# ml-jku/LaM-SLidE

Hardware: AMD Instinct MI355X
Metric: sampled trajectories/sec (50-step ODE) + decoded-coord L2 vs ref, MD17 (higher is better)
Workload: dtype bf16; 1 GPU; md17_bench; tail=False, ln_fuse=True, T=30, L=256, C=32, D=512, H=16, depth=4, sampler=ODE, state_updates=50, batch_per_gpu=32, global_batch=32, parallelism=batch-shard x1, 1 gather to rank 0 per step, noise_elem_stride_per_rank=7864320, kernels=general, trajectories_per_pass=32

## Files before the change

### lam_slide_amd/csrc/k_lin1.hip.h

```cpp
#pragma once
#include <type_traits>

#include "common.hip.h"

struct Lin1Args {
    const u16 *W;
    const u16 *X;
    const float *bias;
    const float4 *rope_q, *rope_k;
    u16 *qkv;
    u16 *z;
    int F, N, HHD, M;
    int pos_div, pos_mod;
    unsigned div_magic, mod_magic;
    float inv_hd, q_premul;
    int nt;
    int wpt;
    int planes;
    int npad;
    const float2 *ln_stat;
    const float *ln_shift, *ln_scale;
    int ln_mod_stride, ln_tpt;
    unsigned ln_tpt_magic;
};

#ifndef LIN1_B2
#define LIN1_B2 1
#endif
#ifndef LIN1_B2_KMAX
#define LIN1_B2_KMAX 256
#endif

template <int HDP, int K, int NW = 8>
struct Lin1Cfg {
    static_assert(K % 128 == 0 && K <= 512, "hidden sizes 128 / 256 / 384 / 512");
    static constexpr int KS = K / 16;
    static constexpr int ROWB = 2 * K;
    static constexpr int PITCH = ROWB + 16;
    static constexpr int BLK = 32 * PITCH;
    static constexpr int NS = (LIN1_B2 && K <= LIN1_B2_KMAX) ? 4 : 3;
    static constexpr int RING = NS * BLK;
    static_assert(NW == 8 || NW == 4, "two waves per SIMD (256-token tiles) or one (128-token tiles)");
    static constexpr int TT = 32 * NW;
    static constexpr int STAGE = NW * 4096;
    static constexpr int LPR = ROWB / 16;
    static constexpr int PPW = 32 / NW;
    static constexpr size_t lds_bytes(int F) { return (size_t)RING + STAGE + (size_t)F * 4; }
    static constexpr int LN_SLOTS = K <= 256 ? 3 : 2;
    static constexpr size_t lds_bytes_lnf(int F) { return lds_bytes(F) + (size_t)LN_SLOTS * 2 * K * 4; }
};

enum { LIN1_QK = 0, LIN1_V = 1, LIN1_MLP = 2 };

#ifndef LIN1_XLOAD
#define LIN1_XLOAD 1
#endif
#ifndef LIN1_PD
#define LIN1_PD 3
#endif

__device__ __forceinline__ float lin1_gelu(float x) {
    const float ax = fabsf(x);
    const float h = __builtin_amdgcn_exp2f(LSL_GELU_Q(ax));
    float relu;
    asm("v_max_f32 %0, 0, %1" : "=v"(relu) : "v"(x));
    return fmaf(-ax, h, relu);
}

template <int HDP, int K, int NW = 8, bool LNF = false>
__global__ void __launch_bounds__(NW * 64, NW / 4) k_linear1_ts(Lin1Args g) {
    using C = Lin1Cfg<HDP, K, NW>;
    constexpr int KS = C::KS, BLK = C::BLK, PPW = C::PPW, ROWB = C::ROWB;
    constexpr int NCO = HDP == 32 ? 8 : 4;
    extern __shared__ __attribute__((aligned(16))) char smem[];

    const int tid = threadIdx.x, lane = tid & 63;
    const int wave = __builtin_amdgcn_readfirstlane(tid >> 6);
    const int r = lane & 31, hf = lane >> 5;
    char *const stage = smem + C::RING + wave * 4096;
    float *const bias_lds = reinterpret_cast<float *>(smem + C::RING + C::STAGE);

    const int NB = g.F >> 5;
    const int ntile = (g.N + C::TT - 1) / C::TT;
    const long U = (long)ntile * NB;
    long i0, i1;
    if (g.wpt > 0) {
        const int tile = blockIdx.x / g.wpt, part = blockIdx.x - tile * g.wpt;
        i0 = (long)tile * NB + ((NB * part / g.wpt) & ~1);
        i1 = (long)tile * NB + (part + 1 == g.wpt ? NB : ((NB * (part + 1) / g.wpt) & ~1));
    } else {
        i0 = (U * blockIdx.x / gridDim.x) & ~1L;
        i1 = blockIdx.x + 1 == gridDim.x ? U : ((U * (blockIdx.x + 1) / gridDim.x) & ~1L);
    }
    if (i0 >= i1) return;

    for (int i = tid * 4; i < g.F; i += NW * 64 * 4) *reinterpret_cast<float4 *>(bias_lds + i) = *reinterpret_cast<const float4 *>(g.bias + i);

    const unsigned lds0 = (unsigned)(size_t)(LDS_PTR(char))(smem);
    const unsigned lane_src = lane * 16;
    const char *const w_rows = reinterpret_cast<const char *>(g.W) + (size_t)(PPW * wave) * ROWB;
    auto issue_piece = [&](const char *src, unsigned dst, auto ic) __attribute__((always_inline)) {
        constexpr int I = decltype(ic)::value & 3;
        if (decltype(ic)::value >= 4) {
            src += 4 * ROWB;
            dst += 4 * C::PITCH;
        }
        const unsigned ls = lane_src;
        if (C::LPR == 64 || lane < C::LPR) {
            if (I == 0 || decltype(ic)::value >= 4)
                asm volatile("s_add_u32 m0, %2, %3\n\ts_nop 4\n\tglobal_load_lds_dwordx4 %0, %1 offset:%4" ::"v"(ls), "s"(src), "s"(dst), "n"(16 * I), "n"(ROWB * I) : "memory", "scc");
            else
                asm volatile("s_add_u32 m0, %2, %3\n\ts_nop 0\n\tglobal_load_lds_dwordx4 %0, %1 offset:%4" ::"v"(ls), "s"(src), "s"(dst), "n"(16 * I), "n"(ROWB * I) : "memory", "scc");
        }
    };
    auto req_src = [&](int blk) __attribute__((always_inline)) { return w_rows + (size_t)blk * (32 * ROWB); };
    auto req_dst = [&](int slot) __attribute__((always_inline)) { return lds0 + slot * BLK + PPW * wave * C::PITCH; };
    auto issue = [&](int blk, int slot) __attribute__((always_inline)) {
        const char *src = req_src(blk);
        const unsigned dst = req_dst(slot);
        issue_piece(src, dst, std::integral_constant<int, 0>());
        issue_piece(src, dst, std::integral_constant<int, 1>());
        issue_piece(src, dst, std::integral_constant<int, 2>());
        issue_piece(src, dst, std::integral_constant<int, 3>());
        if (PPW == 8) {
            issue_piece(src, dst, std::integral_constant<int, 4>());
            issue_piece(src, dst, std::integral_constant<int, 5>());
            issue_piece(src, dst, std::integral_constant<int, 6>());
            issue_piece(src, dst, std::integral_constant<int, 7>());
        }
    };
    const int aoff = r * C::PITCH + 16 * hf;

    bf16x8 xreg[KS];
    float4 co[NCO];
    f32x16 acc0, acc1;
    int slot_c = 0;
    int dma_blk, dma_slot;
    int n_wave = 0;
    float post = 1.0f;

    auto advance = [&](int &b) __attribute__((always_inline)) { b = b + 1 == NB ? 0 : b + 1; };
    auto next_slot = [&](int s) __attribute__((always_inline)) { return s == C::NS - 1 ? 0 : s + 1; };

    {
        int b = (int)(i0 - (i0 / NB) * NB);
        issue(b, 0);
        advance(b);
        issue(b, 1);
        advance(b);
        dma_blk = b;
        dma_slot = 2;
    }

    auto init_acc = [&](f32x16 &a, int blk) __attribute__((always_inline)) {
#pragma unroll
        for (int q4 = 0; q4 < 4; ++q4) {
            const float4 b = *reinterpret_cast<const float4 *>(bias_lds + blk * 32 + 8 * q4 + 4 * hf);
            a[4 * q4] = b.x; a[4 * q4 + 1] = b.y; a[4 * q4 + 2] = b.z; a[4 * q4 + 3] = b.w;
        }
    };
    constexpr bool B2 = LIN1_B2 != 0 && K <= LIN1_B2_KMAX;
    auto step_head = [&](auto flushed_c) __attribute__((always_inline)) {
        if (B2) {
            if (decltype(flushed_c)::value) wait_vmcnt<PPW>();
            else wait_vmcnt<0>();
        } else {
            if (decltype(flushed_c)::value) wait_vmcnt<PPW + 4>();
            else wait_vmcnt<PPW>();
        }
        __builtin_amdgcn_s_barrier();
        asm volatile("" ::: "memory");
    };
    const unsigned wr0 = (unsigned)(size_t)(LDS_PTR(char))(stage) + r * 128 + 8 * hf + ((r & 7) << 4);
    const unsigned rd0 = (unsigned)(size_t)(LDS_PTR(char))(stage) + (lane >> 3) * 128 + (((lane & 7) ^ ((lane >> 3) & 7)) << 4);
    const char *row_q = nullptr, *row_z = nullptr;
    const bool planes = g.planes != 0;
    constexpr unsigned PROW = 2u * HDP, CPH = HDP / 8;
    const unsigned plane_bytes = PROW * (unsigned)g.npad;
    const unsigned stride_q = planes ? PROW : 2u * 3 * g.HHD, stride_z = 2u * (g.HHD + g.M);
    const unsigned blk_q = planes ? (32 / HDP) * plane_bytes : 64u;
    const unsigned voff_q = planes ? ((lane & 7) / CPH) * plane_bytes + (lane >> 3) * PROW + 16 * ((lane & 7) % CPH) : (lane >> 3) * stride_q + 16 * (lane & 7);
    const unsigned voff_z = (lane >> 3) * stride_z + 16 * (lane & 7);
    const int slab_z = 3 * (g.HHD >> 5);
    const char *fl_base = nullptr;
    unsigned fl_stride8 = 0, fl_voff = 0;
    auto flush_setup = [&](int b_even) __attribute__((always_inline)) {
        const bool to_qkv = b_even < slab_z;
        fl_base = to_qkv ? row_q : row_z;
        fl_stride8 = 8 * (to_qkv ? stride_q : stride_z);
        fl_voff = to_qkv ? voff_q + blk_q * (unsigned)b_even : voff_z + 64u * (unsigned)b_even;
    };
    auto flush_read = [&](int half, u32x4 (&pk)[2]) __attribute__((always_inline)) {
#pragma unroll
        for (int i = 0; i < 2; ++i) pk[i] = *reinterpret_cast<const LDS_PTR(u32x4)>(rd0 + 1024 * (2 * half + i));
    };
    auto flush_store = [&](int half, const u32x4 (&pk)[2]) __attribute__((always_inline)) {
        asm volatile("s_nop 4\n\tglobal_store_dwordx4 %0, %1, %2 nt\n\ts_nop 1" ::"v"(fl_voff + (2 * half) * fl_stride8), "v"(pk[0]), "s"(fl_base) : "memory");
        asm volatile("global_store_dwordx4 %0, %1, %2 nt\n\ts_nop 1" ::"v"(fl_voff + (2 * half + 1) * fl_stride8), "v"(pk[1]), "s"(fl_base) : "memory");
    };
    auto flush_store_visible = [&](int half, const u32x4 (&pk)[2]) __attribute__((always_inline)) {
#pragma unroll
        for (int i = 0; i < 2; ++i)
            __builtin_nontemporal_store(pk[i], reinterpret_cast<u32x4 *>(const_cast<char *>(fl_base) + (size_t)(fl_voff + (2 * half + i) * fl_stride8)));
    };
    auto put_group = [&](int ii, int q, float v0, float v1, float v2, float v3) __attribute__((always_inline)) {
        const u32x2 pk = {pack2(v0, v1), pack2(v2, v3)};
        *reinterpret_cast<LDS_PTR(u32x2)>(wr0 ^ (unsigned)(64 * ii + 16 * q)) = pk;
    };
    auto epi_slice = [&](auto sec_c, int s, const f32x16 &a, int ii, float &c0, float &c1) __attribute__((always_inline)) {
        constexpr int SEC = decltype(sec_c)::value;
        if constexpr (SEC == LIN1_QK && HDP == 32) {
            if (s == 0) c0 = 0.0f;
            if (s < 2) {
#pragma unroll
                for (int e = 0; e < 8; ++e) c0 = fmaf(a[8 * s + e], a[8 * s + e], c0);
            }
            if (s == 1) c0 = rsqrtf(fmaf(half_pair_sum(c0), g.inv_hd, 1e-6f)) * post;
            if (s >= 2 && s < 6) {
                const int q = s - 2;
                float o[4];
#pragma unroll
                for (int kk = 0; kk < 2; ++kk) {
                    const int k = 2 * q + kk;
                    const float x0 = a[2 * k], x1 = a[2 * k + 1];
                    o[2 * kk] = c0 * fmaf(co[k].x, x0, -co[k].y * x1);
                    o[2 * kk + 1] = c0 * fmaf(co[k].z, x0, co[k].w * x1);
                }
                put_group(ii, q, o[0], o[1], o[2], o[3]);
            }
        } else if constexpr (SEC == LIN1_QK) {
            if (s == 0) {
                c0 = 0.0f;
#pragma unroll
                for (int e = 0; e < 8; ++e) c0 = fmaf(a[e], a[e], c0);
            }
            if (s == 1) {
                c1 = 0.0f;
#pragma unroll
                for (int e = 0; e < 8; ++e) c1 = fmaf(a[8 + e], a[8 + e], c1);
                c0 = rsqrtf(fmaf(half_pair_sum(c0), g.inv_hd, 1e-6f)) * post;
                c1 = rsqrtf(fmaf(half_pair_sum(c1), g.inv_hd, 1e-6f)) * post;
            }
            if (s >= 2 && s < 6) {
                const int q = s - 2;
                const float rr = q < 2 ? c0 : c1;
                float o[4];
#pragma unroll
                for (int kk = 0; kk < 2; ++kk) {
                    const int k = 2 * q + kk;
                    const float x0 = a[2 * k], x1 = a[2 * k + 1];
                    const float4 cf = co[k & (NCO - 1)];
                    o[2 * kk] = rr * fmaf(cf.x, x0, -cf.y * x1);
                    o[2 * kk + 1] = rr * fmaf(cf.z, x0, cf.w * x1);
                }
                put_group(ii, q, o[0], o[1], o[2], o[3]);
            }
        } else if constexpr (SEC == LIN1_MLP) {
            const float g0 = lin1_gelu(a[2 * s]), g1 = lin1_gelu(a[2 * s + 1]);
            if (s & 1) put_group(ii, s >> 1, c0, c1, g0, g1);
            else { c0 = g0; c1 = g1; }
        } else {
            if (s < 4) put_group(ii, s, a[4 * s], a[4 * s + 1], a[4 * s + 2], a[4 * s + 3]);
        }
    };
    auto step = [&](auto sec_c, auto par_c, auto mfma_c, auto epi_c, auto side) __attribute__((always_inline)) {
        constexpr int PAR = decltype(par_c)::value;
        constexpr bool DO_MFMA = decltype(mfma_c)::value != 0, DO_EPI = decltype(epi_c)::value != 0;
        constexpr int MPS = KS / 8, PD = LIN1_PD, MH = (MPS + 1) / 2;
        f32x16 &ac = PAR ? acc0 : acc1;
        const f32x16 &ae = PAR ? acc1 : acc0;
        const char *sb = smem + slot_c * BLK + aoff;
        bf16x8 fr[PD];
        float c0 = 0.0f, c1 = 0.0f;
        if (DO_MFMA) {
#pragma unroll
            for (int ks = 0; ks < PD; ++ks) fr[ks] = as_bf16x8(*reinterpret_cast<const u32x4 *>(sb + 32 * ks));
        }
        side(std::integral_constant<int, -1>());
#define LIN1_SIDE(S) if (s == S) side(std::integral_constant<int, S>());
#pragma unroll
        for (int s = 0; s < 8; ++s) {
#pragma unroll
            for (int m = 0; m < MPS; ++m) {
                if (m == MH) { LIN1_SIDE(0) LIN1_SIDE(1) LIN1_SIDE(2) LIN1_SIDE(3) LIN1_SIDE(4) LIN1_SIDE(5) LIN1_SIDE(6) LIN1_SIDE(7) }
                if (DO_MFMA) {
                    const int ks = s * MPS + m;
                    ac = mfma32(fr[ks % PD], xreg[ks], ac);
                    if (ks + PD < KS) fr[ks % PD] = as_bf16x8(*reinterpret_cast<const u32x4 *>(sb + 32 * (ks + PD)));
                }
            }
            if (MH == MPS) { LIN1_SIDE(0) LIN1_SIDE(1) LIN1_SIDE(2) LIN1_SIDE(3) LIN1_SIDE(4) LIN1_SIDE(5) LIN1_SIDE(6) LIN1_SIDE(7) }
            if (DO_EPI) epi_slice(sec_c, s, ae, PAR, c0, c1);
            __builtin_amdgcn_sched_barrier(0);
        }
#undef LIN1_SIDE
        if (decltype(mfma_c)::value != 0) slot_c = next_slot(slot_c);
    };
    std::integral_constant<int, 0> I0;
    std::integral_constant<int, 1> I1;
    auto no_side = [](auto) __attribute__((always_inline)) {};
    auto fused = [&](auto sec_c, auto par_c, auto flush_c, auto prev_c, int e) __attribute__((always_inline)) {
        constexpr int PAR = decltype(par_c)::value;
        constexpr bool FLUSH = decltype(flush_c)::value != 0;
        if (!B2 || PAR == 1) step_head(prev_c);
        u32x4 pk[2];
        if (FLUSH) flush_setup(e - 2);
        const char *src = req_src(dma_blk);
        const unsigned dst = req_dst(dma_slot);
        int blk2 = dma_blk;
        advance(blk2);
        const char *src2 = req_src(blk2);
        const unsigned dst2 = req_dst(next_slot(dma_slot));
        init_acc(PAR ? acc0 : acc1, e + 1);
        step(sec_c, par_c, I1, I1, [&](auto sl) __attribute__((always_inline)) {
            constexpr int SL = decltype(sl)::value;
            if (FLUSH) {
                if (SL == -1) flush_read(0, pk);
                if (SL == 0) {
                    flush_store(0, pk);
                    flush_read(1, pk);
                }
                if (SL == 1) flush_store(1, pk);
            }
            constexpr int PS = PPW / 4;
            if (!B2) {
                if (SL >= 2 && SL < 6) {
                    issue_piece(src, dst, std::integral_constant<int, (SL >= 2 && SL < 6) ? PS * (SL - 2) : 0>());
                    if (PS == 2) issue_piece(src, dst, std::integral_constant<int, (SL >= 2 && SL < 6) ? PS * (SL - 2) + 1 : 0>());
                }
            } else if (PAR == 1) {
                if (SL >= 0 && SL < 4) {
                    issue_piece(src, dst, std::integral_constant<int, (SL >= 0 && SL < 4) ? PS * SL : 0>());
                    if (PS == 2) issue_piece(src, dst, std::integral_constant<int, (SL >= 0 && SL < 4) ? PS * SL + 1 : 0>());
                }
                if (SL >= 4 && SL < 8) {
                    issue_piece(src2, dst2, std::integral_constant<int, (SL >= 4 && SL < 8) ? PS * (SL - 4) : 0>());
                    if (PS == 2) issue_piece(src2, dst2, std::integral_constant<int, (SL >= 4 && SL < 8) ? PS * (SL - 4) + 1 : 0>());
                }
            }
        });
        if (!B2) {
            advance(dma_blk);
            dma_slot = next_slot(dma_slot);
        } else if (PAR == 1) {
            advance(dma_blk);
            advance(dma_blk);
            dma_slot = next_slot(next_slot(dma_slot));
        }
    };
    auto run = [&](auto sec_c, int ea, int eb) __attribute__((always_inline)) {
        int e = ea;
        if (e < eb && (e & 1)) {
            fused(sec_c, I1, I0, I0, e);
            ++e;
        }
        for (; e + 1 < eb; e += 2) {
            fused(sec_c, I0, I1, I0, e);
            fused(sec_c, I1, I0, I1, e + 1);
        }
        if (e < eb) fused(sec_c, I0, I1, I0, e);
    };
    auto load_co = [&](const float4 *tab, unsigned pos) __attribute__((always_inline)) {
        const float4 *t = tab + (size_t)pos * (HDP / 2) + 2 * hf;
#pragma unroll
        for (int k = 0; k < NCO; ++k) co[k] = t[4 * (k >> 1) + (k & 1)];
    };
    std::integral_constant<int, LIN1_QK> SQK;
    std::integral_constant<int, LIN1_V> SV;
    std::integral_constant<int, LIN1_MLP> SMLP;

    constexpr bool XLINES = LIN1_XLOAD != 0 && (K <= 384 || LIN1_XLOAD >= 2);
    auto load_x = [&](int nw) __attribute__((always_inline)) {
        if (!XLINES) {
            const u16 *xr = g.X + (size_t)(nw + r) * K + 8 * hf;
#pragma unroll
            for (int ks = 0; ks < KS; ++ks) xreg[ks] = as_bf16x8(*reinterpret_cast<const u32x4 *>(xr + 16 * ks));
        } else {
            const u16 *xr = g.X + (size_t)(nw + (lane >> 3)) * K + 8 * (lane & 7);
#pragma unroll
            for (int j = 0; j < KS / 4; ++j)
#pragma unroll
                for (int q = 0; q < 4; ++q) xreg[4 * j + q] = as_bf16x8(*reinterpret_cast<const u32x4 *>(xr + (size_t)(8 * q) * K + 64 * j));
        }
    };
    auto finish_x = [&]() __attribute__((always_inline)) {
        if (!XLINES) return;
        const unsigned t0 = lane >> 3;
        const unsigned xw = (unsigned)(size_t)(LDS_PTR(char))(stage) + t0 * 128;
        const unsigned xr0 = (unsigned)(size_t)(LDS_PTR(char))(stage) + r * 128;
#pragma unroll
        for (int j = 0; j < KS / 4; ++j) {
#pragma unroll
            for (int q = 0; q < 4; ++q)
                *reinterpret_cast<LDS_PTR(u32x4)>(xw + 1024 * q + ((((lane & 7) ^ ((t0 >> 1) + 4 * q)) & 7) << 4)) = as_u32x4(xreg[4 * j + q]);
#pragma unroll
            for (int m = 0; m < 4; ++m)
                xreg[4 * j + m] = as_bf16x8(*reinterpret_cast<const LDS_PTR(u32x4)>(xr0 + ((((2 * m + hf) ^ (r >> 1)) & 7) << 4)));
        }
    };

    float *const ln_tab = bias_lds + ((g.F + 3) & ~3);
    auto traj_of = [&](unsigned n) __attribute__((always_inline)) { return g.ln_tpt_magic ? __umulhi(n, g.ln_tpt_magic) : n; };
    auto load_x_lnf = [&](int tile_, int nw) __attribute__((always_inline)) {
        typedef __attribute__((ext_vector_type(4))) float f4;
        const float *xf = reinterpret_cast<const float *>(g.X);
        const unsigned t_first = g.ln_mod_stride ? traj_of((unsigned)(tile_ * C::TT)) : 0u;
        const unsigned t_last = g.ln_mod_stride ? traj_of((unsigned)(g.N - 1)) : 0u;
        for (int i = tid * 4; i < C::LN_SLOTS * K; i += NW * 64 * 4) {
            const int slot = i / K, col = i - slot * K;
            const size_t mo = (size_t)min(t_first + (unsigned)slot, t_last) * g.ln_mod_stride + col;
            const f4 sc = *reinterpret_cast<const f4 *>(g.ln_scale + mo), sh = *reinterpret_cast<const f4 *>(g.ln_shift + mo);
            *reinterpret_cast<f4 *>(ln_tab + (size_t)slot * 2 * K + col) = f4{1.0f + sc[0], 1.0f + sc[1], 1.0f + sc[2], 1.0f + sc[3]};
            *reinterpret_cast<f4 *>(ln_tab + (size_t)slot * 2 * K + K + col) = sh;
        }
        const unsigned rowi = lane >> 3, chunk = lane & 7;
        const unsigned sbase = (unsigned)(size_t)(LDS_PTR(char))(stage);
        const unsigned xr0 = sbase + r * 128;
        const float *xr = xf + (size_t)(nw + rowi) * K + 4 * chunk;
        float2 st[4];
        const float *tb[4];
#pragma unroll
        for (int q = 0; q < 4; ++q) {
            const unsigned nn = (unsigned)min(nw + (int)rowi + 8 * q, g.N - 1);
            st[q] = g.ln_stat[nn];
            const unsigned slot = g.ln_mod_stride ? min(traj_of(nn) - t_first, (unsigned)(C::LN_SLOTS - 1)) : 0u;
            tb[q] = ln_tab + (size_t)slot * 2 * K + 4 * chunk;
        }
        __syncthreads();
#pragma unroll
        for (int p = 0; p < K / 64; ++p) {
            f4 v[2][4];
#pragma unroll
            for (int e = 0; e < 2; ++e)
#pragma unroll
                for (int q = 0; q < 4; ++q) v[e][q] = *reinterpret_cast<const f4 *>(xr + (size_t)(8 * q) * K + 64 * p + 32 * e);
#pragma unroll
            for (int q = 0; q < 4; ++q) {
                const unsigned row = rowi + 8 * q, sw = (row >> 1) & 7;
#pragma unroll
                for (int e = 0; e < 2; ++e) {
                    const f4 sc = *reinterpret_cast<const f4 *>(tb[q] + 64 * p + 32 * e), sh = *reinterpret_cast<const f4 *>(tb[q] + K + 64 * p + 32 * e);
                    f4 x = v[e][q];
#pragma unroll
                    for (int c = 0; c < 4; ++c) x[c] = fmaf(x[c], st[q].x, st[q].y) * sc[c] + sh[c];
                    const u32x2 pk = {pack2(x[0], x[1]), pack2(x[2], x[3])};
                    *reinterpret_cast<LDS_PTR(u32x2)>(sbase + row * 128 + ((((4 * e + (chunk >> 1)) ^ sw) & 7) << 4) + 8 * (chunk & 1)) = pk;
                }
            }
#pragma unroll
            for (int m = 0; m < 4; ++m)
                xreg[4 * p + m] = as_bf16x8(*reinterpret_cast<const LDS_PTR(u32x4)>(xr0 + ((((2 * m + hf) ^ (r >> 1)) & 7) << 4)));
            __builtin_amdgcn_sched_barrier(0);
        }
    };
    const int qb = g.HHD >> 5;
    int tile = (int)(i0 / NB), b0 = (int)(i0 - (long)tile * NB), left = (int)(i1 - i0);
    bool first_seg = true;
    bool co_ready = false;
    __syncthreads();
    while (left > 0) {
        const int b1 = NB - b0 < left ? NB : b0 + left;
        n_wave = tile * C::TT + wave * 32;
        row_q = reinterpret_cast<const char *>(g.qkv) + (size_t)n_wave * stride_q;
        row_z = reinterpret_cast<const char *>(g.z) + (size_t)n_wave * stride_z - 4 * (size_t)g.HHD;
        if constexpr (LNF) load_x_lnf(tile, n_wave);
        else {
            if (first_seg) load_x(n_wave);
            finish_x();
        }
        const unsigned nn = (unsigned)min(n_wave + r, g.N - 1);
        const unsigned n1 = g.div_magic ? __umulhi(nn, g.div_magic) : nn;
        const unsigned pos = g.mod_magic ? n1 - __umulhi(n1, g.mod_magic) * (unsigned)g.pos_mod : 0u;

        if (first_seg) wait_vmcnt<0>();
        else wait_vmcnt<4>();
        __builtin_amdgcn_s_barrier();
        asm volatile("" ::: "memory");
        issue(dma_blk, dma_slot);
        advance(dma_blk);
        dma_slot = next_slot(dma_slot);
        if (B2) {
            issue(dma_blk, dma_slot);
            advance(dma_blk);
            dma_slot = next_slot(dma_slot);
        }
        init_acc(acc0, b0);
        step(SV, I1, I1, I0, no_side);
        const int e_end = b1 - 1;
        if (b0 < 2 * qb) {
            if (!co_ready) load_co(b0 < qb ? g.rope_q : g.rope_k, pos);
            post = b0 < qb ? g.q_premul : 1.0f;
            fused(SQK, I0, I0, I0, b0);
        } else if (b0 < 3 * qb) {
            fused(SV, I0, I0, I0, b0);
        } else {
            fused(SMLP, I0, I0, I0, b0);
        }
        {
            const int lo = max(b0 + 1, 0), hi = min(e_end, qb);
            if (lo < hi) run(SQK, lo, hi);
        }
        {
            const int lo = max(b0 + 1, qb), hi = min(e_end, 2 * qb);
            if (lo < hi) {
                if (lo == qb) {
                    load_co(g.rope_k, pos);
                    post = 1.0f;
                }
                run(SQK, lo, hi);
            }
        }
        {
            const int lo = max(b0 + 1, 2 * qb), hi = min(e_end, 3 * qb);
            if (lo < hi) run(SV, lo, hi);
        }
        {
            const int lo = max(b0 + 1, 3 * qb), hi = min(e_end, NB);
            if (lo < hi) run(SMLP, lo, hi);
        }
        const int left_next = left - (b1 - b0);
        co_ready = false;
        if (left_next > 0) {
            asm volatile("" ::: "memory");
            const int nw = (tile + 1) * C::TT + wave * 32;
            if constexpr (!LNF) load_x(nw);
            if (b1 - 1 >= 2 * qb) {
                const unsigned nn2 = (unsigned)min(nw + r, g.N - 1);
                const unsigned m1 = g.div_magic ? __umulhi(nn2, g.div_magic) : nn2;
                load_co(g.rope_q, g.mod_magic ? m1 - __umulhi(m1, g.mod_magic) * (unsigned)g.pos_mod : 0u);
                co_ready = true;
            }
            asm volatile("" ::: "memory");
        }
        {
            const int e = b1 - 1;
            if (e < 2 * qb) {
                step(SQK, I1, I0, I1, no_side);
            } else if (e < 3 * qb) {
                step(SV, I1, I0, I1, no_side);
            } else {
                step(SMLP, I1, I0, I1, no_side);
            }
            flush_setup(e - 1);
            u32x4 pk[2];
            flush_read(0, pk);
            flush_store_visible(0, pk);
            flush_read(1, pk);
            flush_store_visible(1, pk);
        }
        left = left_next;
        tile += 1;
        b0 = 0;
        first_seg = false;
    }
    wait_vmcnt<0>();
}
```

Baseline: 57.81 trajectories/s.

## Defer last-block output flush into next tile's first step in LN-fused linear1

When layernorm fusion is active, the final block's output flush of a tile is no longer done serially at the end. It is postponed and interleaved into the first MFMA step of the next tile, using the DMA ring slot as LDS staging for the normalized X. The wait counts are adjusted to match. The LN table reads are also changed to LDS-pointer arithmetic with precomputed swizzle offsets. The aim is to hide the store tail behind compute, at the cost of stricter waits (vmcnt(0) plus lgkmcnt(0)) at tile boundaries and extra control complexity.

```diff
diff --git a/lam_slide_amd/csrc/k_lin1.hip.h b/lam_slide_amd/csrc/k_lin1.hip.h
--- a/lam_slide_amd/csrc/k_lin1.hip.h
+++ b/lam_slide_amd/csrc/k_lin1.hip.h
@@ -58,6 +58,9 @@
 #ifndef LIN1_PD
 #define LIN1_PD 3
 #endif
+#ifndef LIN1_LNF_DEFER
+#define LIN1_LNF_DEFER 1
+#endif
 
 __device__ __forceinline__ float lin1_gelu(float x) {
     const float ax = fabsf(x);
@@ -160,12 +163,17 @@
         }
     };
     constexpr bool B2 = LIN1_B2 != 0 && K <= LIN1_B2_KMAX;
+    constexpr bool DEFER = LNF && LIN1_LNF_DEFER != 0 && NW == 8 && (B2 ? 2 : 1) * BLK >= NW * 4096;
+    bool pending = false;
     auto step_head = [&](auto flushed_c) __attribute__((always_inline)) {
         if (B2) {
             if (decltype(flushed_c)::value) wait_vmcnt<PPW>();
             else wait_vmcnt<0>();
         } else {
-            if (decltype(flushed_c)::value) wait_vmcnt<PPW + 4>();
+            if constexpr (decltype(flushed_c)::value == 2) {
+                if (pending) wait_vmcnt<PPW + 4>();
+                else wait_vmcnt<PPW>();
+            } else if (decltype(flushed_c)::value) wait_vmcnt<PPW + 4>();
             else wait_vmcnt<PPW>();
         }
         __builtin_amdgcn_s_barrier();
@@ -190,6 +198,14 @@
         fl_stride8 = 8 * (to_qkv ? stride_q : stride_z);
         fl_voff = to_qkv ? voff_q + blk_q * (unsigned)b_even : voff_z + 64u * (unsigned)b_even;
     };
+    auto flush_setup_prev = [&]() __attribute__((always_inline)) {
+        const int b_even = NB - 2;
+        const bool to_qkv = b_even < slab_z;
+        const unsigned stride = to_qkv ? stride_q : stride_z;
+        fl_base = (to_qkv ? row_q : row_z) - (size_t)C::TT * stride;
+        fl_stride8 = 8 * stride;
+        fl_voff = to_qkv ? voff_q + blk_q * (unsigned)b_even : voff_z + 64u * (unsigned)b_even;
+    };
     auto flush_read = [&](int half, u32x4 (&pk)[2]) __attribute__((always_inline)) {
 #pragma unroll
         for (int i = 0; i < 2; ++i) pk[i] = *reinterpret_cast<const LDS_PTR(u32x4)>(rd0 + 1024 * (2 * half + i));
@@ -197,6 +213,11 @@
     auto flush_store = [&](int half, const u32x4 (&pk)[2]) __attribute__((always_inline)) {
         asm volatile("s_nop 4\n\tglobal_store_dwordx4 %0, %1, %2 nt\n\ts_nop 1" ::"v"(fl_voff + (2 * half) * fl_stride8), "v"(pk[0]), "s"(fl_base) : "memory");
         asm volatile("global_store_dwordx4 %0, %1, %2 nt\n\ts_nop 1" ::"v"(fl_voff + (2 * half + 1) * fl_stride8), "v"(pk[1]), "s"(fl_base) : "memory");
+    };
+    auto flush_store_sbase = [&](int half, const u32x4 (&pk)[2]) __attribute__((always_inline)) {
+#pragma unroll
+        for (int i = 0; i < 2; ++i)
+            asm volatile("s_nop 4\n\tglobal_store_dwordx4 %0, %1, %2 nt\n\ts_nop 1" ::"v"(fl_voff), "v"(pk[i]), "s"(fl_base + (size_t)(2 * half + i) * fl_stride8) : "memory");
     };
     auto flush_store_visible = [&](int half, const u32x4 (&pk)[2]) __attribute__((always_inline)) {
 #pragma unroll
@@ -414,19 +435,21 @@
             *reinterpret_cast<f4 *>(ln_tab + (size_t)slot * 2 * K + K + col) = sh;
         }
         const unsigned rowi = lane >> 3, chunk = lane & 7;
-        const unsigned sbase = (unsigned)(size_t)(LDS_PTR(char))(stage);
-        const unsigned xr0 = sbase + r * 128;
+        const unsigned sbase = DEFER ? lds0 + (unsigned)dma_slot * BLK + (unsigned)wave * 4096u : (unsigned)(size_t)(LDS_PTR(char))(stage);
+        const unsigned xr0 = sbase + r * 128, xu = ((hf ^ (r >> 1)) & 7) << 4;
+        const unsigned xw0 = sbase + rowi * 128 + ((((chunk >> 1) ^ (rowi >> 1)) & 3) << 4) + 8 * (chunk & 1);
         const float *xr = xf + (size_t)(nw + rowi) * K + 4 * chunk;
         float2 st[4];
-        const float *tb[4];
+        unsigned tb[4];
+        const unsigned tab0 = (unsigned)(size_t)(LDS_PTR(char))(reinterpret_cast<char *>(ln_tab)) + 16 * chunk;
+        __syncthreads();
 #pragma unroll
         for (int q = 0; q < 4; ++q) {
             const unsigned nn = (unsigned)min(nw + (int)rowi + 8 * q, g.N - 1);
             st[q] = g.ln_stat[nn];
             const unsigned slot = g.ln_mod_stride ? min(traj_of(nn) - t_first, (unsigned)(C::LN_SLOTS - 1)) : 0u;
-            tb[q] = ln_tab + (size_t)slot * 2 * K + 4 * chunk;
-        }
-        __syncthreads();
+            tb[q] = tab0 + slot * (2 * K * 4);
+        }
 #pragma unroll
         for (int p = 0; p < K / 64; ++p) {
             f4 v[2][4];
@@ -439,17 +462,17 @@
                 const unsigned row = rowi + 8 * q, sw = (row >> 1) & 7;
 #pragma unroll
                 for (int e = 0; e < 2; ++e) {
-                    const f4 sc = *reinterpret_cast<const f4 *>(tb[q] + 64 * p + 32 * e), sh = *reinterpret_cast<const f4 *>(tb[q] + K + 64 * p + 32 * e);
+                    const f4 sc = *reinterpret_cast<const LDS_PTR(f4)>(tb[q] + 4 * (64 * p + 32 * e)), sh = *reinterpret_cast<const LDS_PTR(f4)>(tb[q] + 4 * (K + 64 * p + 32 * e));
                     f4 x = v[e][q];
 #pragma unroll
                     for (int c = 0; c < 4; ++c) x[c] = fmaf(x[c], st[q].x, st[q].y) * sc[c] + sh[c];
                     const u32x2 pk = {pack2(x[0], x[1]), pack2(x[2], x[3])};
-                    *reinterpret_cast<LDS_PTR(u32x2)>(sbase + row * 128 + ((((4 * e + (chunk >> 1)) ^ sw) & 7) << 4) + 8 * (chunk & 1)) = pk;
+                    *reinterpret_cast<LDS_PTR(u32x2)>(xw0 + 1024 * q + 64 * (e ^ (q & 1))) = pk;
                 }
             }
 #pragma unroll
             for (int m = 0; m < 4; ++m)
-                xreg[4 * p + m] = as_bf16x8(*reinterpret_cast<const LDS_PTR(u32x4)>(xr0 + ((((2 * m + hf) ^ (r >> 1)) & 7) << 4)));
+                xreg[4 * p + m] = as_bf16x8(*reinterpret_cast<const LDS_PTR(u32x4)>(xr0 + (xu ^ (unsigned)(32 * m))));
             __builtin_amdgcn_sched_barrier(0);
         }
     };
@@ -472,8 +495,9 @@
         const unsigned n1 = g.div_magic ? __umulhi(nn, g.div_magic) : nn;
         const unsigned pos = g.mod_magic ? n1 - __umulhi(n1, g.mod_magic) * (unsigned)g.pos_mod : 0u;
 
-        if (first_seg) wait_vmcnt<0>();
+        if (first_seg || DEFER) wait_vmcnt<0>();
         else wait_vmcnt<4>();
+        if constexpr (DEFER) asm volatile("s_waitcnt lgkmcnt(0)" ::: "memory");
         __builtin_amdgcn_s_barrier();
         asm volatile("" ::: "memory");
         issue(dma_blk, dma_slot);
@@ -485,17 +509,35 @@
             dma_slot = next_slot(dma_slot);
         }
         init_acc(acc0, b0);
-        step(SV, I1, I1, I0, no_side);
+        bool flush_prev = false;
+        if constexpr (DEFER) flush_prev = pending;
+        if (flush_prev) {
+            flush_setup_prev();
+            u32x4 pk[2];
+            step(SV, I1, I1, I0, [&](auto sl) __attribute__((always_inline)) {
+                constexpr int SL = decltype(sl)::value;
+                if (SL == -1) flush_read(0, pk);
+                if (SL == 0) {
+                    flush_store_sbase(0, pk);
+                    flush_read(1, pk);
+                }
+                if (SL == 1) flush_store_sbase(1, pk);
+            });
+        } else {
+            step(SV, I1, I1, I0, no_side);
+        }
+        std::integral_constant<int, DEFER ? 2 : 0> PV;
         const int e_end = b1 - 1;
         if (b0 < 2 * qb) {
             if (!co_ready) load_co(b0 < qb ? g.rope_q : g.rope_k, pos);
             post = b0 < qb ? g.q_premul : 1.0f;
-            fused(SQK, I0, I0, I0, b0);
+            fused(SQK, I0, I0, PV, b0);
         } else if (b0 < 3 * qb) {
-            fused(SV, I0, I0, I0, b0);
+            fused(SV, I0, I0, PV, b0);
         } else {
-            fused(SMLP, I0, I0, I0, b0);
-        }
+            fused(SMLP, I0, I0, PV, b0);
+        }
+        pending = false;
         {
             const int lo = max(b0 + 1, 0), hi = min(e_end, qb);
             if (lo < hi) run(SQK, lo, hi);
@@ -541,12 +583,18 @@
             } else {
                 step(SMLP, I1, I0, I1, no_side);
             }
-            flush_setup(e - 1);
-            u32x4 pk[2];
-            flush_read(0, pk);
-            flush_store_visible(0, pk);
-            flush_read(1, pk);
-            flush_store_visible(1, pk);
+            bool defer_now = false;
+            if constexpr (DEFER) defer_now = left_next > 0;
+            if (defer_now) {
+                pending = true;
+            } else {
+                flush_setup(e - 1);
+                u32x4 pk[2];
+                flush_read(0, pk);
+                flush_store_visible(0, pk);
+                flush_read(1, pk);
+                flush_store_visible(1, pk);
+            }
         }
         left = left_next;
         tile += 1;
```

Measured after the change: 57.76 trajectories/s. About the same (-0.1%).
